# sisl/NeRFSafetyValidation

Measured on AMD Instinct MI355X. Metric: rendered_samples_per_sec, higher is better.
Workload: dtype f16; 1 GPU; Stonehenge 800x800 synthetic, hashgrid L=16 F=2 T=2^19 + ffmlp(64,2)/(64,3), fp16, occupancy-grid ray marching (run_cuda eval path, BASELINE configs[1]); rays_per_frame=640000, bound=2, cascade=2, frames_in_flight=3, fused_reference_rounding=True, parallelism=single GPU, rccl_ranks=1

## Files before the change

include/ngp_hip.h:

```cpp
#ifndef NGP_HIP_H
#define NGP_HIP_H

#include <stddef.h>
#include <stdint.h>

#ifdef __cplusplus
extern "C" {
#endif

#define NGP_OK 0
#define NGP_EINVAL (-1)
#define NGP_ELAUNCH (-2)
#define NGP_EWORKSPACE (-3)
#define NGP_ENODEVICE (-4)

#define NGP_F32 0
#define NGP_F16 1

typedef void* ngp_stream_t;

#if defined(NGP_BUILD)
#define NGP_API __attribute__((visibility("default")))
#else
#define NGP_API
// ... 246 lines not shown

NGP_API int ngp_adam_advance_step(float* step_dev, const float* found_inf_dev, ngp_stream_t stream);
NGP_API int ngp_adam_step_dev(float* param, const float* grad, float* exp_avg, float* exp_avg_sq, uint64_t n, float lr, float beta1,
                      float beta2, float eps, const float* step_dev, const float* grad_scale_dev, const float* found_inf_dev,
                      ngp_stream_t stream);

NGP_API size_t ngp_sift_workspace(uint32_t H, uint32_t W);
NGP_API size_t ngp_sift_layer_offset(uint32_t H, uint32_t W, int octave, int index);
NGP_API int ngp_sift_octaves(uint32_t H, uint32_t W);
NGP_API int ngp_sift_interest_mask(const uint8_t* rgb, uint32_t H, uint32_t W, uint32_t kernel_size, uint32_t dil_iter, uint8_t* points,
                                   uint8_t* mask, uint32_t* count, void* workspace, size_t workspace_bytes, ngp_stream_t stream);

NGP_API int ngp_debug_set_stamps(unsigned long long* device_buf);
NGP_API int ngp_debug_set_sample_hash(uint32_t* device_buf);
NGP_API int ngp_debug_disable_march_queue(int off);
NGP_API int ngp_debug_fused_features(const ngp_model* model, const float* xyzs, uint32_t M, int operator_rounding, uint16_t* features,
                             ngp_stream_t stream);
NGP_API int ngp_debug_set_grad_dump(float* device_buf);
NGP_API int ngp_render_ctx_set_debug(ngp_render_ctx* ctx, int enable, int flags, unsigned long long* stamps, uint32_t* sample_hash);

NGP_API int ngp_prof_enable(int on);
NGP_API int ngp_prof_reset(void);
NGP_API int ngp_prof_read(const char* name, double* total_ms, uint64_t* launches, double* units);

#ifdef __cplusplus
}
#endif
#endif
```

nerfsafetyvalidation_amd/_lib.py:

```python
import ctypes as C
import os

import torch

_HERE = os.path.dirname(os.path.abspath(__file__))
SO_PATH = os.environ.get("NGP_HIP_LIB", os.path.join(_HERE, "libngp_hip.so"))

NGP_F32, NGP_F16 = 0, 1
NGP_PREC_F16, NGP_PREC_F32, NGP_PREC_F16_REF = 0, 1, 2
NGP_EDT_INF = 0x7FFFFFFF

_vp, _u32, _f32, _int, _sz = C.c_void_p, C.c_uint32, C.c_float, C.c_int, C.c_size_t


class ModelStruct(C.Structure):
    _fields_ = [
        ("embeddings", _vp), ("offsets_host", _vp), ("L", _u32), ("S", _f32), ("H_base", _u32), ("gridtype", _u32),
        ("align_corners", _int), ("sigma_weights", _vp), ("sigma_hidden_mm", _u32), ("color_weights", _vp),
        ("color_hidden_mm", _u32), ("bound", _f32), ("density_scale", _f32), ("density_bitfield", _vp),
        ("cascade", _u32), ("grid_size", _u32), ("cell_tables", _vp), ("cell_levels", _u32), ("packed_weights", _vp),
        ("precision", _u32),
    ]


# ... 85 lines not shown
    "ngp_transmittance_weights": [_vp, _vp, _vp, _u32, _u32, _f32, _vp, _vp],
    "ngp_transmittance_weights_backward": [_vp, _vp, _vp, _vp, _u32, _u32, _f32, _vp, _vp],
    "ngp_sample_pdf": [_vp, _vp, _u32, _u32, _vp, _int, _u32, _vp, _vp],
    "ngp_merge_sorted": [_vp, _vp, _u32, _u32, _u32, _vp, _vp, _vp],
    "ngp_mark_untrained_grid": [_vp, _u32, _f32, _f32, _f32, _f32, _f32, _u32, _u32, _vp, _vp, _sz, _vp],
    "ngp_density_grid_points": [_vp, _u32, _u32, _f32, _vp, _vp, _vp, _vp],
    "ngp_density_grid_workspace": [_u32, _u32],
    "ngp_density_grid_update": [_vp, _u32, _u32, _u32, _vp, _vp, _u32, _f32, _f32, _vp, _sz, _vp],
    "ngp_density_grid_finish": [_vp, _u32, _u32, _f32, _vp, _vp, _vp, _sz, _vp],
    "ngp_render_uniform": [C.POINTER(ModelStruct), _vp, _vp, _vp, _vp, _u32, _u32, _vp, _vp, _vp, _vp, _vp, _u32, _vp, _vp, _u32, _vp],
    "ngp_render_upsample": [C.POINTER(ModelStruct), _vp, _vp, _vp, _vp, _u32, _u32, _u32, _vp, _vp, _vp, _vp, _vp, _vp, _u32, _vp, _vp, _u32, _vp, _sz, _vp],
    "ngp_render_upsample_workspace": [_u32, _u32, _u32],
    "ngp_debug_set_stamps": [_vp],
    "ngp_debug_set_sample_hash": [_vp],
    "ngp_debug_disable_march_queue": [_int],
    "ngp_render_ctx_set_debug": [_vp, _int, _int, _vp, _vp],
    "ngp_debug_set_grad_dump": [_vp],
    "ngp_debug_fused_features": [C.POINTER(ModelStruct), _vp, _u32, _int, _vp, _vp],
    "ngp_prof_enable": [_int],
    "ngp_prof_reset": [],
    "ngp_prof_read": [C.c_char_p, C.POINTER(C.c_double), C.POINTER(C.c_uint64), C.POINTER(C.c_double)],
}
_RESTYPES = {"ngp_render_uniform_backward_lds": _sz, "ngp_cell_tables_bytes": _sz, "ngp_packed_weights_bytes": _sz, "ngp_packed_weights_bwd_bytes": _sz, "ngp_grid_encode_backward_workspace": _sz,
             "ngp_ffmlp_backward_workspace": _sz, "ngp_ffmlp_backward_buffer_bytes": _sz, "ngp_render_upsample_workspace": _sz, "ngp_density_grid_workspace": _sz, "ngp_last_error": C.c_char_p, "ngp_march_rays_train_workspace": _sz, "ngp_uq_stats_workspace": _sz, "ngp_occupancy_lin_bytes": _sz, "ngp_edt_sq_workspace": _sz, "ngp_sift_workspace": _sz, "ngp_sift_layer_offset": _sz}

_lib = None


def lib():
    global _lib
# ... 59 lines not shown
```

nerfsafetyvalidation_amd/csrc/fused_net.hpp:

```cpp
#pragma once
#include <hip/hip_fp16.h>
#include <math.h>

#include "ngp_common.hpp"

namespace ngp {

typedef _Float16 half8 __attribute__((ext_vector_type(8)));
typedef _Float16 half2v __attribute__((ext_vector_type(2)));
typedef _Float16 half4 __attribute__((ext_vector_type(4)));
typedef float f32x4 __attribute__((ext_vector_type(4)));

struct LevelTab {
    float scale[16];
    uint32_t offset[16], size[16];
    uint32_t a1[16], a2[16];
    uint32_t mask[16];
    uint32_t flags[16];
    uint32_t cell_off[16], cell_res[16];
};

struct NetArgs {
    const uint32_t* table;
    const _Float16* packed;
// ... 859 lines not shown
struct DebugState {
    int flags = 0;
    unsigned long long* stamps = nullptr;
    uint32_t* sample_hash = nullptr;
    bool coarse_off() const { return (flags & 2) != 0; }
    bool sort_off() const { return (flags & 4) != 0; }
    bool lin_off() const { return (flags & 8) != 0; }
    bool jump_off() const { return (flags & 1) != 0; }
    bool spec_off() const { return (flags & 256) != 0; }
    bool tile_off() const { return (flags & 8192) != 0; }
    bool pre_verdict_off() const { return (flags & 16384) != 0; }
    bool narrow_items_off() const { return (flags & 32768) != 0; }
    bool prefix_replay_off() const { return (flags & 65536) != 0; }
    bool wave_march_off() const { return (flags & 131072) != 0; }
    bool cell_runs_off() const { return (flags & 262144) != 0; }
    uint32_t spec_safety_x2() const { return ((uint32_t)flags >> 9) & 15u; }
    uint32_t shrink() const { return ((uint32_t)flags >> 4) & 15u; }
};
DebugState debug_snapshot();
float* grad_dump();
bool needs_generic(const GridLevels& lv);
int fill_net(const ngp_model* m, const DebugState& dbg, const _Float16* packed, NetArgs& na, GridLevels& lv);
size_t weights_bytes(const NetArgs& na);
uint32_t resident_blocks(size_t lds);
int net_variant(const NetArgs& na, const GridLevels& lv);
bool bwd_shape_ok(const NetArgs& na);
#define NGP_WITH_NET(variant, ...)                                           \
    switch (variant) {                                                       \
        case 0: { using NET = NetF16<0>; __VA_ARGS__; } break;               \
        case 1: { using NET = NetF16<1>; __VA_ARGS__; } break;               \
// ... 10 lines not shown
```

nerfsafetyvalidation_amd/csrc/ngp_common.hpp:

```cpp
#pragma once
#include <hip/hip_runtime.h>
#include <stdint.h>
#include <stdio.h>
#include <string>

#include "../../include/ngp_hip.h"

namespace ngp {

void set_error(const char* fmt, ...);
int check_launch(const char* what);

#define NGP_REQUIRE(cond, ...)                 \
    do {                                       \
        if (!(cond)) {                         \
            ngp::set_error(__VA_ARGS__);       \
            return NGP_EINVAL;                 \
        }                                      \
    } while (0)

struct ProfScope {
    ProfScope(const char* name, hipStream_t s, double units);
    ~ProfScope();
    int slot;
// ... 8 lines not shown

constexpr int kMaxLevels = 32;
struct GridLevels {
    float scale[kMaxLevels];
    uint32_t resolution[kMaxLevels];
    uint32_t offset[kMaxLevels + 1];
    uint32_t mul1[kMaxLevels], mul2[kMaxLevels];
    uint8_t hashed[kMaxLevels], mode[kMaxLevels];
};
void fill_levels(GridLevels& lv, const int32_t* offsets_host, uint32_t L, float S, uint32_t H, uint32_t D, uint32_t gridtype,
                 bool align_corners);

__global__ void k_build_linear(const uint8_t* __restrict__ bitfield, uint32_t cascade, uint32_t logH, uint32_t* __restrict__ lin);
__global__ void k_build_coarse_linear(const unsigned long long* __restrict__ bitfield64, uint32_t cascade, uint32_t logH,
                                      unsigned long long* __restrict__ coarse);
constexpr size_t kTrainLinBytes = 1u << 20;
constexpr size_t kTrainCoarseBytes = 8192;

__device__ __forceinline__ _Float16 mul_round_f16(float w, _Float16 g) {
    float p = w * (float)g;
    asm volatile("" : "+v"(p));
    return (_Float16)p;
}
__device__ __forceinline__ float clampf(float x, float lo, float hi) { return fminf(hi, fmaxf(lo, x)); }
__device__ __forceinline__ float signf(float x) { return copysignf(1.0f, x); }

__device__ __forceinline__ uint32_t expand_bits(uint32_t v) {
    v = (v * 0x00010001u) & 0xFF0000FFu;
    v = (v * 0x00000101u) & 0x0F00F00Fu;
    v = (v * 0x00000011u) & 0xC30C30C3u;
    v = (v * 0x00000005u) & 0x49249249u;
    return v;
}
__device__ __forceinline__ uint32_t morton3D(uint32_t x, uint32_t y, uint32_t z) {
    return expand_bits(x) | (expand_bits(y) << 1) | (expand_bits(z) << 2);
}
__device__ __forceinline__ uint32_t expand_bits10(uint32_t v) {
    v = (v | (v << 16)) & 0xFF0000FFu;
    v = (v | (v << 8)) & 0x0F00F00Fu;
    v = (v | (v << 4)) & 0xC30C30C3u;
    v = (v | (v << 2)) & 0x49249249u;
    return v;
}
__device__ __forceinline__ uint32_t morton3D_cell(uint32_t x, uint32_t y, uint32_t z) {
    return expand_bits10(x) | (expand_bits10(y) << 1) | (expand_bits10(z) << 2);
}
__device__ __forceinline__ uint32_t morton3D_invert(uint32_t x) {
    x = x & 0x49249249u;
    x = (x | (x >> 2)) & 0xc30c30c3u;
    x = (x | (x >> 4)) & 0x0f00f00fu;
    x = (x | (x >> 8)) & 0xff0000ffu;
    x = (x | (x >> 16)) & 0x0000ffffu;
    return x;
}

struct Pcg32 {
    uint64_t state, inc;
    __host__ __device__ uint32_t next_uint() {
        const uint64_t old = state;
// ... 28 lines not shown
};

struct Dda {
    float ox, oy, oz, dx, dy, dz, rdx, rdy, rdz;
    float bound, rbound, dt_gamma, dt_min, dt_max, dt_c, rH, H3f, Cf, Hf, Hm1, halfH;
    double Hd;
    bool h_pow2, const_dt;
    int level_dt0;
    float t_fast_min;
    const uint32_t* grid_lin;
    uint32_t logH;
    int sx, sy, sz;
    float two_rH;
    float jump_guard;
    bool block_jump;
    const uint8_t* grid;

    __device__ __forceinline__ void init(const float* o, const float* d, const uint8_t* g, float bound_, float dt_gamma_,
                                         uint32_t max_steps, uint32_t C, uint32_t H) {
        ox = o[0]; oy = o[1]; oz = o[2];
        dx = d[0]; dy = d[1]; dz = d[2];
        rdx = 1 / dx; rdy = 1 / dy; rdz = 1 / dz;
        rH = 1 / (float)H;
        H3f = (float)(H * H * H);
        bound = bound_; rbound = 1 / bound_; dt_gamma = dt_gamma_;
        const float SQRT3 = 1.7320508075688772f;
        dt_min = 2 * SQRT3 / (float)max_steps;
        dt_max = 2 * SQRT3 * (float)(1 << (C - 1)) / (float)H;
        Cf = (float)C; Hf = (float)H; Hm1 = (float)(H - 1); Hd = (double)H;
        h_pow2 = (H & (H - 1)) == 0;
        halfH = 0.5f * Hf;
        grid = g;
        const_dt = dt_gamma_ == 0.0f;
        dt_c = fminf(dt_max, fmaxf(0.0f, dt_min));
        level_dt0 = mip_from_dt(dt_c);
        const uint32_t b = __float_as_uint(dt_c);
        const uint32_t m = (b & 0x7FFFFFu) | 0x800000u;
        t_fast_min = __uint_as_float(((b >> 23) + (uint32_t)__ffs((int)m) + 1u) << 23);
    }

    __device__ __forceinline__ void init_lin(const uint32_t* lin, uint32_t logH_, bool block_jump_) {
        grid_lin = lin;
        block_jump = block_jump_;
        logH = logH_;
        sx = (int)((__float_as_uint(dx) >> 31) ^ 1u);
        sy = (int)((__float_as_uint(dy) >> 31) ^ 1u);
        sz = (int)((__float_as_uint(dz) >> 31) ^ 1u);
        two_rH = 2.0f * rH;
        jump_guard = bound * 9.5367431640625e-7f;
    }

    __device__ __forceinline__ void skip_const_dt(float& t, float tt) const {
        const float t1 = t + dt_c;
        if (!(t1 < tt)) { t = t1; return; }
        const float d = t1 - t;
        const float r = tt - t1;
        float t2 = fmaf(ceilf(r * __builtin_amdgcn_rcpf(d)), d, t1);
        if (t2 < tt) t2 += d;
// ... 52 lines not shown
        mip_bound = use_pw ? pw : bound;
        const float mip_rbound = use_pw ? __uint_as_float((uint32_t)(127 - level) << 23) : rbound;
        nx = cell_pow2(x, mip_rbound); ny = cell_pow2(y, mip_rbound); nz = cell_pow2(z, mip_rbound);
    }
    __device__ __forceinline__ uint32_t coarse_index_lin(int level, int nx, int ny, int nz) const {
        const uint32_t lb = logH - 2;
        return ((uint32_t)level << (3 * lb)) + ((((uint32_t)nz >> 2) << (2 * lb)) | (((uint32_t)ny >> 2) << lb) | ((uint32_t)nx >> 2));
    }
    __device__ __forceinline__ bool coarse_empty_at_lin(float t, const uint32_t* coarse) const {
        float x, y, z, dt, mip_bound;
        int level, nx, ny, nz;
        locate_lin(t, x, y, z, dt, level, mip_bound, nx, ny, nz);
        const uint32_t ci = coarse_index_lin(level, nx, ny, nz);
        return ((coarse[ci >> 5] >> (ci & 31u)) & 1u) == 0;
    }
    __device__ __forceinline__ bool jump_block(float& t, float x, float y, float z, int level, float mip_bound, int nx, int ny, int nz) const {
        const float bx = fmaf((float)((nx & ~3) + 4 * sx), two_rH, -1.0f), by = fmaf((float)((ny & ~3) + 4 * sy), two_rH, -1.0f),
                    bz = fmaf((float)((nz & ~3) + 4 * sz), two_rH, -1.0f);
        if (level > level_dt0) {
            if (mip_bound != (float)(1 << level)) return false;
            const float cell4 = 4.0f * two_rH;
            const float ox_ = sx ? bx - cell4 : bx, oy_ = sy ? by - cell4 : by, oz_ = sz ? bz - cell4 : bz;
            const float mx = (ox_ <= 0.0f && ox_ + cell4 >= 0.0f) ? 0.0f : fminf(fabsf(ox_), fabsf(ox_ + cell4));
            const float my = (oy_ <= 0.0f && oy_ + cell4 >= 0.0f) ? 0.0f : fminf(fabsf(oy_), fabsf(oy_ + cell4));
            const float mz = (oz_ <= 0.0f && oz_ + cell4 >= 0.0f) ? 0.0f : fminf(fabsf(oz_), fabsf(oz_ + cell4));
            if (fmaxf(mx, fmaxf(my, mz)) < 0.5f) return false;
        }
        const float tx = fmaf(bx, mip_bound, -x) * rdx, ty = fmaf(by, mip_bound, -y) * rdy, tz = fmaf(bz, mip_bound, -z) * rdz;
        const float tmin = fminf(tx, fminf(ty, tz));
        const float tt = t + fmaxf(0.0f, tmin);
        const float t1 = t + dt_c;
        if (!(t1 < tt)) return false;
        const float d = t1 - t;
        float t2 = fmaf(ceilf((tt - t1) * __builtin_amdgcn_rcpf(d)), d, t1);
        if (t2 < tt) t2 += d;
        else if (t2 - d >= tt) t2 -= d;
        const float ex = fabsf(rdx) * jump_guard, ey = fabsf(rdy) * jump_guard, ez = fabsf(rdz) * jump_guard;
        const float em = tmin == tx ? ex : (tmin == ty ? ey : ez);
        const float lim = tmin + em;
        float ga = em;
        if (tx - ex <= lim) ga = fmaxf(ga, ex);
        if (ty - ey <= lim) ga = fmaxf(ga, ey);
        if (tz - ez <= lim) ga = fmaxf(ga, ez);
        const float guard = fmaf(t2, 9.5367431640625e-7f, ga);
        const bool clear = (t2 - tt) > guard && (tt - (t2 - d)) > guard;
        const bool same_binade = ((__float_as_uint(t2) ^ __float_as_uint(t)) >> 23) == 0;
        if (!(clear && same_binade && t >= t_fast_min)) return false;
        t = t2;
        return true;
    }

    __device__ __forceinline__ bool probe_lin(float& t, float& x, float& y, float& z, float& dt, const uint32_t* coarse,
                                              float* occupied_until = nullptr) const {
        float mip_bound;
        int level, nx, ny, nz;
        locate_lin(t, x, y, z, dt, level, mip_bound, nx, ny, nz);
        const uint32_t ci = coarse_index_lin(level, nx, ny, nz);
        bool occ = false;
        if ((coarse[ci >> 5] >> (ci & 31u)) & 1u) {
            const uint32_t fi = ((uint32_t)level << (3 * logH)) + (((uint32_t)nz << (2 * logH)) | ((uint32_t)ny << logH) | (uint32_t)nx);
            occ = ((grid_lin[fi >> 5] >> (fi & 31u)) & 1u) != 0;
            if (occ && occupied_until) {
                const float tx = fmaf(fmaf((float)(nx + sx), two_rH, -1.0f), mip_bound, -x) * rdx;
                const float ty = fmaf(fmaf((float)(ny + sy), two_rH, -1.0f), mip_bound, -y) * rdy;
                const float tz = fmaf(fmaf((float)(nz + sz), two_rH, -1.0f), mip_bound, -z) * rdz;
                const float tt = t + fminf(tx, fminf(ty, tz));
                const float g = fmaf(tt, 9.5367431640625e-7f, (fabsf(rdx) + fabsf(rdy) + fabsf(rdz)) * jump_guard);
                const float until = tt - g;
                *occupied_until = until > t ? until : t;
            }
        } else if (const_dt && block_jump && jump_block(t, x, y, z, level, mip_bound, nx, ny, nz)) {
            return false;
        }
        if (!occ) {
            const float tx = fmaf(fmaf((float)(nx + sx), two_rH, -1.0f), mip_bound, -x) * rdx;
            const float ty = fmaf(fmaf((float)(ny + sy), two_rH, -1.0f), mip_bound, -y) * rdy;
            const float tz = fmaf(fmaf((float)(nz + sz), two_rH, -1.0f), mip_bound, -z) * rdz;
            const float tt = t + fmaxf(0.0f, fminf(tx, fminf(ty, tz)));
            if (const_dt) {
                skip_const_dt(t, tt);
            } else {
                do { t += clampf(t * dt_gamma, dt_min, dt_max); } while (t < tt);
            }
        }
        return occ;
    }

// ... 33 lines not shown
```

nerfsafetyvalidation_amd/csrc/render_fused.hip:

```cpp
#include <hip/hip_fp16.h>
#include <math.h>
#include <string.h>

#include <atomic>

#include "fused_net.hpp"

namespace ngp {

constexpr int kWaves = 8;
constexpr int kThreads = kWaves * 64;
constexpr int kWavesPerSimd = 4;
constexpr int kCh = 2;
constexpr int kSlots = 64 * kCh;
constexpr size_t kLinMaxBytes = 4u << 20;
constexpr size_t kCoarseMaxBytes = 8192;
constexpr int kLookahead = 4;
constexpr int kRing = 8;

struct Ctl {
    uint32_t n_alive, n_step, step, done;
    uint32_t iters, last_n_alive, last_n_step, pad;
    unsigned long long samples_marched, samples_slots;
    uint32_t spec, rollbacks, backoff, rsv;
// ... 37 lines not shown
    lin[w] = out;
}

__global__ void __launch_bounds__(256) k_build_coarse_linear(const unsigned long long* __restrict__ bitfield64, uint32_t cascade, uint32_t logH,
                                                             unsigned long long* __restrict__ coarse) {
    const uint32_t i = blockIdx.x * 256 + threadIdx.x;
    const uint32_t lb = logH - 2, per_level = 1u << (3 * lb), B1 = (1u << lb) - 1;
    bool any = false;
    if (i < cascade * per_level) {
        const uint32_t level = i / per_level, r = i % per_level;
        const uint32_t bx = r & B1, by = (r >> lb) & B1, bz = r >> (2 * lb);
        any = bitfield64[(size_t)level * per_level + morton3D_cell(bx, by, bz)] != 0ull;
    }
    const unsigned long long m = __ballot(any);
    if ((threadIdx.x & 63) == 0 && i < cascade * per_level) coarse[i >> 6] = m;
}

struct RenderArgs {
    const float *rays_o, *rays_d, *fars;
    float* rays_t;
    float *weights_sum, *depth, *image;
    float *last_sigmas, *last_rgbs;
    float pad_sigma, pad_r, pad_g, pad_b;
    float4* dump_rec;
    uint32_t* dump_iter;
    const int32_t* alive_in;
    int32_t* staging;
    uint32_t* chunk_count;
    uint32_t sort_slow;
    Ctl* ctl;
    QueueHeads* heads;
    unsigned long long* stat_shards;
    uint32_t* death_shards;
    float4* backup;
    const uint8_t* bitfield;
    uint32_t cascade, grid_size, max_steps, perturb;
    float dt_gamma;
    Pcg32 rng;
    const uint32_t* coarse;
    uint32_t coarse_words;
    const uint32_t* bitfield_lin;
    uint32_t log_grid;
    uint32_t block_jump;
    uint32_t* sample_hash;
    unsigned long long* stamps;
    float2* march_samples;
    uint8_t* march_counts;
    uint32_t wave_slots;
    uint32_t n_rays;
    uint32_t pre_verdict;
    uint32_t wave_march_max;
    uint32_t cell_runs;
};

__host__ __device__ __forceinline__ uint32_t item_width(uint32_t n_alive, uint32_t wave_slots) {
    return n_alive >= 64u * wave_slots ? 64u : (n_alive >= 32u * wave_slots ? 32u : 16u);
}
__device__ __forceinline__ void truncate_launch(Ctl& c, const uint32_t* exhausted, uint32_t N) {
// ... 32 lines not shown
    } else {
        const size_t row = (size_t)entry * n_step + k;
        ra.last_sigmas[row] = sg;
        ra.last_rgbs[row * 3] = r; ra.last_rgbs[row * 3 + 1] = g; ra.last_rgbs[row * 3 + 2] = b;
    }
}

__device__ __forceinline__ void march_ahead_wave(const RenderArgs& ra, float bound, const Ctl& ctl, const uint32_t* coarse) {
    const uint32_t lane = threadIdx.x & 63u;
    const uint32_t entry = blockIdx.x * 4u + (threadIdx.x >> 6);
    if (entry >= ctl.n_alive) return;
    const uint32_t n_step = ctl.n_step, spec = ctl.spec;
    const int32_t ray = ra.alive_in[entry];
    Dda dda;
    dda.init(ra.rays_o + (size_t)ray * 3, ra.rays_d + (size_t)ray * 3, ra.bitfield, bound, 0.0f, ra.max_steps, ra.cascade, ra.grid_size);
    dda.init_lin(ra.bitfield_lin, ra.log_grid, ra.block_jump != 0);
    const float t_c = ra.rays_t[ray], far = ra.fars[ray];
    float t_march = t_c;
    if (ra.perturb) {
        Pcg32 rng = ra.rng;
        rng.advance((int64_t)entry);
        t_march += dda.dt_min * rng.next_float();
    }
    float last_m = t_march, geo_tc = t_c;
    uint32_t emitted = 0, rounds = 0;
    float2* out = ra.march_samples + ((size_t)(entry >> 6) * n_step) * 64 + (entry & 63u);
    while (t_march < far && emitted < n_step) {
        rounds++;
        const float t1 = t_march + dda.dt_c, d = t1 - t_march;
        const float p = lane == 0 ? t_march : fmaf((float)lane, d, t_march);
        const bool exact = t_march >= dda.t_fast_min && ((__float_as_uint(p) ^ __float_as_uint(t_march)) >> 23) == 0;
// ... 57 lines not shown
    const bool by_wave = LIN && n_alive <= ra.wave_march_max;
    if (blockIdx.x * (by_wave ? 4u : 256u) >= n_alive) return;
    __shared__ uint32_t coarse_lds[kCoarseMaxBytes / 4];
    for (uint32_t i = threadIdx.x; i < ra.coarse_words; i += blockDim.x) coarse_lds[i] = ra.coarse[i];
    __syncthreads();
    const uint32_t* coarse = ra.coarse_words ? coarse_lds : nullptr;
    if (LIN && by_wave) {
        march_ahead_wave(ra, bound, ctl, coarse);
        return;
    }
    const uint32_t entry = blockIdx.x * blockDim.x + threadIdx.x;
    if (entry >= n_alive) return;
    const int32_t ray = ra.alive_in[entry];
    Dda dda;
    dda.init(ra.rays_o + (size_t)ray * 3, ra.rays_d + (size_t)ray * 3, ra.bitfield, bound, ra.dt_gamma, ra.max_steps, ra.cascade, ra.grid_size);
    if (LIN) dda.init_lin(ra.bitfield_lin, ra.log_grid, ra.block_jump != 0);
    const float t_c = ra.rays_t[ray], far = ra.fars[ray];
    float t_march = t_c;
    if (ra.perturb) {
        Pcg32 rng = ra.rng;
        rng.advance((int64_t)entry);
        t_march += dda.dt_min * rng.next_float();
    }
    float last_m = t_march;
    float geo_tc = t_c;
    uint32_t emitted = 0;
    float2* out = ra.march_samples + ((size_t)(entry >> 6) * n_step) * 64 + (entry & 63u);
    float x, y, z, dt;
    uint32_t probes = 0, probes_coarse_empty = 0, probes_fine_empty = 0;
    const bool run_cells = LIN && dda.const_dt && ra.cell_runs != 0;
    float occ_until = 0.0f;
    while (t_march < far && emitted < n_step) {
        probes++;
        const bool diag_ce = LIN && ra.stamps && dda.coarse_empty_at_lin(t_march, coarse);
        const uint32_t emitted_before = emitted;
        if (LIN ? dda.probe_lin(t_march, x, y, z, dt, coarse, run_cells ? &occ_until : nullptr) : dda.probe(t_march, x, y, z, dt, coarse)) {
            do {
                out[(size_t)emitted * 64] = make_float2(t_march, dt);
                t_march += dt;
                const float d1 = t_march - last_m;
                last_m = t_march;
                geo_tc += d1;
                emitted++;
                if (spec && emitted % spec == 0) {
                    t_march = geo_tc;
                    last_m = geo_tc;
                }
            } while (run_cells && t_march < occ_until && t_march < far && emitted < n_step);
        }
        if (ra.stamps && emitted == emitted_before) { if (diag_ce) probes_coarse_empty++; else probes_fine_empty++; }
    }
// ... 5 lines not shown
            mx = mx > o ? mx : o;
            sm += p2;
        }
        if ((threadIdx.x & 63u) == (uint32_t)__builtin_ctzll(__ballot(true))) {
            atomicAdd(ra.stamps + 4, (unsigned long long)mx);
            atomicAdd(ra.stamps + 5, (unsigned long long)sm);
            atomicAdd(ra.stamps + 6, 1ull);
            atomicMax(ra.stamps + 7, (unsigned long long)mx);
        }
        uint32_t ce = probes_coarse_empty, fe = probes_fine_empty;
#pragma unroll
        for (int off = 32; off > 0; off >>= 1) { ce += (uint32_t)__shfl_xor((int)ce, off, 64); fe += (uint32_t)__shfl_xor((int)fe, off, 64); }
        if ((threadIdx.x & 63u) == (uint32_t)__builtin_ctzll(__ballot(true))) {
            atomicAdd(ra.stamps + 14, (unsigned long long)ce);
            atomicAdd(ra.stamps + 15, (unsigned long long)fe);
        }
    }
    if (spec && ra.pre_verdict) {
        const uint32_t K = n_step / spec, jd = emitted < n_step ? emitted / spec : 0xFFFFFFFFu;
        const unsigned long long act = __ballot(true);
        const bool leader = (threadIdx.x & 63u) == (uint32_t)__builtin_ctzll(act);
        uint32_t* ex = ra.death_shards + (size_t)kDeathShards * kSpecK + (blockIdx.x % kDeathShards) * kSpecK;
        for (uint32_t j = 0; j < K; j++) {
            const unsigned long long b = __ballot(jd == j);
            if (leader && b) atomicAdd(&ex[j], (uint32_t)__popcll(b));
        }
    }
    bool slow = false;
    if (ra.sort_slow && emitted == n_step) slow = geo_tc < far && (LIN ? dda.coarse_empty_at_lin(geo_tc, coarse) : dda.coarse_empty_at(geo_tc, coarse));
    ra.march_counts[entry] = (uint8_t)(emitted | (slow ? 128u : 0u));
// ... 581 lines not shown
}

}

using namespace ngp;

struct ngp_render_ctx {
    uint32_t max_rays = 0;
    uint32_t frame_width = 0;
    int32_t* alive[2] = {nullptr, nullptr};
    int32_t* staging = nullptr;
    uint32_t* chunk_count = nullptr;
    float* rays_t = nullptr;
    unsigned long long* coarse = nullptr;
    uint32_t* grid_lin = nullptr;
    uint32_t* death_shards = nullptr;
    float4* backup = nullptr;
    float2* march_samples = nullptr;
    uint8_t* march_counts = nullptr;
    float4* dump_rec = nullptr;
    uint32_t* dump_iter = nullptr;
    Ctl* ctl = nullptr;
    unsigned long long* stat_shards = nullptr;
    QueueHeads* heads = nullptr;
    _Float16* packed = nullptr;
    unsigned long long* status = nullptr;
    unsigned long long* status_dev = nullptr;
    unsigned long long* fin = nullptr;
    unsigned long long* fin_dev = nullptr;
    uint32_t calls = 0;
// ... 25 lines not shown
    const size_t chunks = div_up(max_rays, 64);
    bool ok = true;
    int cus = 256;
    {
        int dev = 0;
        hipDeviceProp_t prop;
        if (hipGetDevice(&dev) == hipSuccess && hipGetDeviceProperties(&prop, dev) == hipSuccess) cus = prop.multiProcessorCount;
    }
    const size_t max_items = items_bound(max_rays, (uint32_t)cus * 16u) + 8;
    ok &= hipMalloc(&c->alive[0], (size_t)max_rays * 4) == hipSuccess;
    ok &= hipMalloc(&c->alive[1], (size_t)max_rays * 4) == hipSuccess;
    ok &= hipMalloc(&c->staging, chunks * 64 * 4) == hipSuccess;
    ok &= hipMalloc(&c->chunk_count, (max_items > (size_t)div_up(max_rays, 256) ? max_items : (size_t)div_up(max_rays, 256)) * 4) == hipSuccess;
    ok &= hipMalloc(&c->rays_t, (size_t)max_rays * 4) == hipSuccess;
    ok &= hipMalloc(&c->coarse, kCoarseMaxBytes) == hipSuccess;
    ok &= hipMalloc(&c->ctl, 2 * sizeof(Ctl)) == hipSuccess;
    ok &= hipMalloc(&c->stat_shards, kStatShards * sizeof(unsigned long long)) == hipSuccess;
    ok &= hipMalloc(&c->death_shards, 2 * (size_t)kDeathWords * sizeof(uint32_t)) == hipSuccess;
    ok &= hipMalloc(&c->backup, (size_t)max_rays * 2 * sizeof(float4)) == hipSuccess;
    ok &= hipMalloc(&c->march_samples, ((size_t)max_rays + 512) * 8 * sizeof(float2)) == hipSuccess;
    ok &= hipMalloc(&c->march_counts, (size_t)max_rays) == hipSuccess;
    ok &= hipMalloc(&c->heads, 2 * sizeof(QueueHeads)) == hipSuccess;
    ok &= hipMalloc(&c->packed, (size_t)(sig_halfs(2) + sig_halfs(3)) * 2) == hipSuccess;
    ok &= hipHostMalloc(&c->status, kRing * sizeof(unsigned long long), hipHostMallocMapped | hipHostMallocCoherent) == hipSuccess;
    if (ok) {
        memset(c->status, 0, kRing * sizeof(unsigned long long));
        ok &= hipHostGetDevicePointer((void**)&c->status_dev, c->status, 0) == hipSuccess;
    }
    ok &= hipHostMalloc(&c->fin, 4 * sizeof(unsigned long long), hipHostMallocMapped | hipHostMallocCoherent) == hipSuccess;
    if (ok) {
// ... 11 lines not shown
    }
    *out = c;
    return NGP_OK;
}

int ngp_render_ctx_set_frame_width(ngp_render_ctx* ctx, uint32_t width) {
    NGP_REQUIRE(ctx, "render_ctx_set_frame_width: null context");
    ctx->frame_width = width;
    return NGP_OK;
}

int ngp_render_ctx_destroy(ngp_render_ctx* c) {
    if (!c) return NGP_OK;
    (void)hipDeviceSynchronize();
    (void)hipFree(c->alive[0]); (void)hipFree(c->alive[1]); (void)hipFree(c->staging); (void)hipFree(c->chunk_count);
    (void)hipFree(c->rays_t); (void)hipFree(c->coarse); (void)hipFree(c->grid_lin); (void)hipFree(c->death_shards); (void)hipFree(c->backup); (void)hipFree(c->march_samples); (void)hipFree(c->march_counts); (void)hipFree(c->dump_rec); (void)hipFree(c->dump_iter); (void)hipFree(c->ctl); (void)hipFree(c->stat_shards); (void)hipFree(c->heads); (void)hipFree(c->packed);
    if (c->status) (void)hipHostFree(c->status);
    if (c->fin) (void)hipHostFree(c->fin);
    for (int i = 0; i < kRing; i++) (void)hipEventDestroy(c->ev[i]);
    delete c;
    return NGP_OK;
}

static std::atomic<int> g_active_renders{0};
struct ActiveRender {
    ActiveRender() { g_active_renders.fetch_add(1, std::memory_order_relaxed); }
    ~ActiveRender() { g_active_renders.fetch_sub(1, std::memory_order_relaxed); }
};

int ngp_render_rays(ngp_render_ctx* ctx, const ngp_model* model, const float* rays_o, const float* rays_d, const float* nears,
                    const float* fars, uint32_t N, float dt_gamma, uint32_t max_steps, uint32_t perturb, float* weights_sum, float* depth,
// ... 62 lines not shown
    const uint32_t Hg = model->grid_size;
    uint32_t logH = 0;
    while ((1u << logH) < Hg) logH++;
    bool lin = use_coarse && !dbg.lin_off() && (1u << logH) == Hg && Hg >= 8 && cells / 8 <= kLinMaxBytes;
    if (lin && !ctx->grid_lin && hipMalloc(&ctx->grid_lin, kLinMaxBytes) != hipSuccess) lin = false;
    if (lin) {
        const uint32_t n_words = (uint32_t)(cells / 32), n_coarse = (uint32_t)(cells / 64);
        k_build_linear<<<div_up(n_words, 256), 256, 0, s>>>(model->density_bitfield, model->cascade, logH, ctx->grid_lin);
        k_build_coarse_linear<<<div_up(n_coarse, 256), 256, 0, s>>>((const unsigned long long*)model->density_bitfield, model->cascade, logH,
                                                                     ctx->coarse);
        ra.coarse = (const uint32_t*)ctx->coarse;
        ra.coarse_words = (uint32_t)(coarse_bytes / 4);
        ra.bitfield_lin = ctx->grid_lin;
        ra.log_grid = logH;
        ra.block_jump = dbg.jump_off() ? 0u : 1u;
    } else if (use_coarse) {
        const uint32_t n_words = (uint32_t)(cells / 64);
        k_build_coarse<<<div_up(n_words, 256), 256, 0, s>>>((const unsigned long long*)model->density_bitfield, n_words, ctx->coarse);
        ra.coarse = (const uint32_t*)ctx->coarse;
        ra.coarse_words = (uint32_t)(coarse_bytes / 4);
    } else {
        ra.sort_slow = 0;
    }
    if ((ra.sort_slow || tile_w) && last_sigmas) {
        if (!ctx->dump_rec) {
            if (hipMalloc(&ctx->dump_rec, (size_t)ctx->max_rays * 8 * sizeof(float4)) != hipSuccess ||
                hipMalloc(&ctx->dump_iter, (size_t)ctx->max_rays * 4) != hipSuccess) {
                set_error("render_rays: cannot allocate the per-ray record buffer");
                return NGP_ENODEVICE;
            }
// ... 139 lines not shown
        if (stats_host) {
            stats_host->samples_marched = fin.samples_marched;
            stats_host->samples_slots = fin.samples_slots;
            stats_host->iterations = fin.iters;
            stats_host->rays = N;
            stats_host->last_n_alive = fin.last_n_alive;
            stats_host->last_n_step = fin.last_n_step;
            stats_host->launches = launches;
            stats_host->replayed = fin.rollbacks;
            prof_add_units("k_render_iter", (double)fin.samples_marched);
        }
    }
    return NGP_OK;
}

int ngp_render_ctx_set_debug(ngp_render_ctx* ctx, int enable, int flags, unsigned long long* stamps, uint32_t* sample_hash) {
    NGP_REQUIRE(ctx, "render_ctx_set_debug: null context");
    ctx->has_debug = enable != 0;
    ctx->debug_flags = flags;
    ctx->debug_stamps = stamps;
    ctx->debug_sample_hash = sample_hash;
    return NGP_OK;
}

}
```

Measured before the change: 7.621 billion samples/s.

## Add empty-space radius map for wide block jumps in constant-dt ray marching

After: 7.581 billion samples/s. Within noise of the previous version (-0.5%).

```diff
diff --git a/include/ngp_hip.h b/include/ngp_hip.h
--- a/include/ngp_hip.h
+++ b/include/ngp_hip.h
@@ -284,6 +284,8 @@
 NGP_API int ngp_debug_set_stamps(unsigned long long* device_buf);
 NGP_API int ngp_debug_set_sample_hash(uint32_t* device_buf);
 NGP_API int ngp_debug_disable_march_queue(int off);
+NGP_API int ngp_debug_empty_radius(const uint8_t* bitfield, uint32_t cascade, uint32_t grid_size, uint8_t* radius, int on_host,
+                                   ngp_stream_t stream);
 NGP_API int ngp_debug_fused_features(const ngp_model* model, const float* xyzs, uint32_t M, int operator_rounding, uint16_t* features,
                              ngp_stream_t stream);
 NGP_API int ngp_debug_set_grad_dump(float* device_buf);
diff --git a/nerfsafetyvalidation_amd/_lib.py b/nerfsafetyvalidation_amd/_lib.py
--- a/nerfsafetyvalidation_amd/_lib.py
+++ b/nerfsafetyvalidation_amd/_lib.py
@@ -123,6 +123,7 @@
     "ngp_debug_set_stamps": [_vp],
     "ngp_debug_set_sample_hash": [_vp],
     "ngp_debug_disable_march_queue": [_int],
+    "ngp_debug_empty_radius": [_vp, _u32, _u32, _vp, _int, _vp],
     "ngp_render_ctx_set_debug": [_vp, _int, _int, _vp, _vp],
     "ngp_debug_set_grad_dump": [_vp],
     "ngp_debug_fused_features": [C.POINTER(ModelStruct), _vp, _u32, _int, _vp, _vp],
diff --git a/nerfsafetyvalidation_amd/csrc/fused_net.hpp b/nerfsafetyvalidation_amd/csrc/fused_net.hpp
--- a/nerfsafetyvalidation_amd/csrc/fused_net.hpp
+++ b/nerfsafetyvalidation_amd/csrc/fused_net.hpp
@@ -897,6 +897,7 @@
     bool prefix_replay_off() const { return (flags & 65536) != 0; }
     bool wave_march_off() const { return (flags & 131072) != 0; }
     bool cell_runs_off() const { return (flags & 262144) != 0; }
+    bool wide_jump_off() const { return (flags & 524288) != 0; }
     uint32_t spec_safety_x2() const { return ((uint32_t)flags >> 9) & 15u; }
     uint32_t shrink() const { return ((uint32_t)flags >> 4) & 15u; }
 };
diff --git a/nerfsafetyvalidation_amd/csrc/ngp_common.hpp b/nerfsafetyvalidation_amd/csrc/ngp_common.hpp
--- a/nerfsafetyvalidation_amd/csrc/ngp_common.hpp
+++ b/nerfsafetyvalidation_amd/csrc/ngp_common.hpp
@@ -46,6 +46,60 @@
 __global__ void k_build_linear(const uint8_t* __restrict__ bitfield, uint32_t cascade, uint32_t logH, uint32_t* __restrict__ lin);
 __global__ void k_build_coarse_linear(const unsigned long long* __restrict__ bitfield64, uint32_t cascade, uint32_t logH,
                                       unsigned long long* __restrict__ coarse);
+constexpr int kEmptyRadiusMax = 7;
+__host__ __device__ __forceinline__ uint32_t radius_row_bits(const uint32_t* coarse, uint32_t level, uint32_t lb, uint32_t by, uint32_t bz) {
+    const uint32_t B = 1u << lb;
+    const uint32_t base = (level << (3 * lb)) + (((bz << lb) | by) << lb);
+    uint32_t row = (coarse[base >> 5] >> (base & 31u)) & (uint32_t)((1ull << B) - 1ull);
+    if (level > 0 && 4u * (by + 1u) > B && 4u * by < 3u * B && 4u * (bz + 1u) > B && 4u * bz < 3u * B) {
+        const uint32_t lo = B / 4u, hi = (3u * B + 3u) / 4u;
+        row |= (uint32_t)(((1ull << hi) - 1ull) & ~((1ull << lo) - 1ull));
+    }
+    return row;
+}
+__host__ __device__ __forceinline__ uint32_t radius_row_dist(uint32_t row, uint32_t lb, uint32_t bx) {
+    const uint32_t B = 1u << lb, cap = (uint32_t)kEmptyRadiusMax + 1u;
+    if ((row >> bx) & 1u) return 0u;
+    const uint32_t below = row & ((1u << bx) - 1u), above = (row >> bx) >> 1;
+    const uint32_t dl = below ? bx - (31u - (uint32_t)__builtin_clz(below)) : bx + 1u;
+    const uint32_t dr = above ? (uint32_t)__builtin_ctz(above) + 1u : B - bx;
+    const uint32_t d = dl < dr ? dl : dr;
+    return d < cap ? d : cap;
+}
+__host__ __device__ __forceinline__ uint32_t radius_pass_xy(const uint32_t* coarse, uint32_t lb, uint32_t i) {
+    const uint32_t B1 = (1u << lb) - 1u, cap = (uint32_t)kEmptyRadiusMax + 1u;
+    const uint32_t level = i >> (3 * lb), bx = i & B1, by = (i >> lb) & B1, bz = (i >> (2 * lb)) & B1;
+    uint32_t best = cap;
+    for (int k = -kEmptyRadiusMax; k <= kEmptyRadiusMax; k++) {
+        const uint32_t ak = (uint32_t)(k < 0 ? -k : k);
+        const int y = (int)by + k;
+        uint32_t c = ak;
+        if (y >= 0 && y <= (int)B1) {
+            const uint32_t dx = radius_row_dist(radius_row_bits(coarse, level, lb, (uint32_t)y, bz), lb, bx);
+            c = dx > ak ? dx : ak;
+        }
+        best = c < best ? c : best;
+    }
+    return best;
+}
+__host__ __device__ __forceinline__ uint32_t radius_pass_z(const uint8_t* xy, uint32_t lb, uint32_t i) {
+    const uint32_t B1 = (1u << lb) - 1u, cap = (uint32_t)kEmptyRadiusMax + 1u;
+    const uint32_t bz = (i >> (2 * lb)) & B1;
+    uint32_t best = cap;
+    for (int k = -kEmptyRadiusMax; k <= kEmptyRadiusMax; k++) {
+        const uint32_t ak = (uint32_t)(k < 0 ? -k : k);
+        const int z = (int)bz + k;
+        uint32_t c = ak;
+        if (z >= 0 && z <= (int)B1) {
+            const uint32_t d = xy[(size_t)((int)i + k * (int)(1u << (2 * lb)))];
+            c = d > ak ? d : ak;
+        }
+        best = c < best ? c : best;
+    }
+    return best ? best - 1u : 0u;
+}
+__global__ void k_build_radius_xy(const uint32_t* __restrict__ coarse, uint32_t cascade, uint32_t logH, uint8_t* __restrict__ xy);
+__global__ void k_build_radius_z(const uint8_t* __restrict__ xy, uint32_t cascade, uint32_t logH, uint32_t* __restrict__ radius);
 constexpr size_t kTrainLinBytes = 1u << 20;
 constexpr size_t kTrainCoarseBytes = 8192;
 
@@ -67,14 +121,14 @@
 __device__ __forceinline__ uint32_t morton3D(uint32_t x, uint32_t y, uint32_t z) {
     return expand_bits(x) | (expand_bits(y) << 1) | (expand_bits(z) << 2);
 }
-__device__ __forceinline__ uint32_t expand_bits10(uint32_t v) {
+__host__ __device__ __forceinline__ uint32_t expand_bits10(uint32_t v) {
     v = (v | (v << 16)) & 0xFF0000FFu;
     v = (v | (v << 8)) & 0x0F00F00Fu;
     v = (v | (v << 4)) & 0xC30C30C3u;
     v = (v | (v << 2)) & 0x49249249u;
     return v;
 }
-__device__ __forceinline__ uint32_t morton3D_cell(uint32_t x, uint32_t y, uint32_t z) {
+__host__ __device__ __forceinline__ uint32_t morton3D_cell(uint32_t x, uint32_t y, uint32_t z) {
     return expand_bits10(x) | (expand_bits10(y) << 1) | (expand_bits10(z) << 2);
 }
 __device__ __forceinline__ uint32_t morton3D_invert(uint32_t x) {
@@ -133,6 +187,7 @@
     float two_rH;
     float jump_guard;
     bool block_jump;
+    const uint32_t* radius;
     const uint8_t* grid;
 
     __device__ __forceinline__ void init(const float* o, const float* d, const uint8_t* g, float bound_, float dt_gamma_,
@@ -158,9 +213,10 @@
         t_fast_min = __uint_as_float(((b >> 23) + (uint32_t)__ffs((int)m) + 1u) << 23);
     }
 
-    __device__ __forceinline__ void init_lin(const uint32_t* lin, uint32_t logH_, bool block_jump_) {
+    __device__ __forceinline__ void init_lin(const uint32_t* lin, uint32_t logH_, bool block_jump_, const uint32_t* radius_ = nullptr) {
         grid_lin = lin;
         block_jump = block_jump_;
+        radius = radius_;
         logH = logH_;
         sx = (int)((__float_as_uint(dx) >> 31) ^ 1u);
         sy = (int)((__float_as_uint(dy) >> 31) ^ 1u);
@@ -243,12 +299,14 @@
         const uint32_t ci = coarse_index_lin(level, nx, ny, nz);
         return ((coarse[ci >> 5] >> (ci & 31u)) & 1u) == 0;
     }
-    __device__ __forceinline__ bool jump_block(float& t, float x, float y, float z, int level, float mip_bound, int nx, int ny, int nz) const {
-        const float bx = fmaf((float)((nx & ~3) + 4 * sx), two_rH, -1.0f), by = fmaf((float)((ny & ~3) + 4 * sy), two_rH, -1.0f),
-                    bz = fmaf((float)((nz & ~3) + 4 * sz), two_rH, -1.0f);
+    __device__ __forceinline__ bool jump_block(float& t, float x, float y, float z, int level, float mip_bound, int nx, int ny, int nz,
+                                               int R = 0) const {
+        const int lo = 4 * R, span = 4 + 8 * R;
+        const float bx = fmaf((float)((nx & ~3) - lo + span * sx), two_rH, -1.0f), by = fmaf((float)((ny & ~3) - lo + span * sy), two_rH, -1.0f),
+                    bz = fmaf((float)((nz & ~3) - lo + span * sz), two_rH, -1.0f);
         if (level > level_dt0) {
             if (mip_bound != (float)(1 << level)) return false;
-            const float cell4 = 4.0f * two_rH;
+            const float cell4 = (float)span * two_rH;
             const float ox_ = sx ? bx - cell4 : bx, oy_ = sy ? by - cell4 : by, oz_ = sz ? bz - cell4 : bz;
             const float mx = (ox_ <= 0.0f && ox_ + cell4 >= 0.0f) ? 0.0f : fminf(fabsf(ox_), fabsf(ox_ + cell4));
             const float my = (oy_ <= 0.0f && oy_ + cell4 >= 0.0f) ? 0.0f : fminf(fabsf(oy_), fabsf(oy_ + cell4));
@@ -278,9 +336,20 @@
         t = t2;
         return true;
     }
+    __device__ __forceinline__ int fit_radius(int R, float t, float x, float y, float z, float mip_bound, int nx, int ny, int nz) const {
+        const float tx = fmaf(fmaf((float)((nx & ~3) + 4 * sx), two_rH, -1.0f), mip_bound, -x) * rdx;
+        const float ty = fmaf(fmaf((float)((ny & ~3) + 4 * sy), two_rH, -1.0f), mip_bound, -y) * rdy;
+        const float tz = fmaf(fmaf((float)((nz & ~3) + 4 * sz), two_rH, -1.0f), mip_bound, -z) * rdz;
+        const float tb = __uint_as_float((__float_as_uint(t) & 0x7F800000u) + 0x00800000u);
+        const float room = (tb - t) - 2.0f * dt_c;
+        const float blocks = fmaxf(fmaxf((room - tx) * fabsf(dx), (room - ty) * fabsf(dy)), (room - tz) * fabsf(dz)) *
+                             __builtin_amdgcn_rcpf(4.0f * two_rH * mip_bound);
+        const int fit = (int)fmaxf(blocks, 0.0f);
+        return fit < R ? fit : R;
+    }
 
     __device__ __forceinline__ bool probe_lin(float& t, float& x, float& y, float& z, float& dt, const uint32_t* coarse,
-                                              float* occupied_until = nullptr) const {
+                                              float* occupied_until = nullptr, uint32_t* wide_stats = nullptr) const {
         float mip_bound;
         int level, nx, ny, nz;
         locate_lin(t, x, y, z, dt, level, mip_bound, nx, ny, nz);
@@ -298,8 +367,18 @@
                 const float until = tt - g;
                 *occupied_until = until > t ? until : t;
             }
-        } else if (const_dt && block_jump && jump_block(t, x, y, z, level, mip_bound, nx, ny, nz)) {
-            return false;
+        } else if (const_dt && block_jump) {
+            int R = radius ? (int)((radius[ci >> 3] >> ((ci & 7u) * 4u)) & 15u) : 0;
+            if (R) R = fit_radius(R, t, x, y, z, mip_bound, nx, ny, nz);
+            for (;;) {
+                if (jump_block(t, x, y, z, level, mip_bound, nx, ny, nz, R)) {
+                    if (wide_stats && R) wide_stats[0]++;
+                    return false;
+                }
+                if (R == 0) break;
+                if (wide_stats) wide_stats[1]++;
+                R = 0;
+            }
         }
         if (!occ) {
             const float tx = fmaf(fmaf((float)(nx + sx), two_rH, -1.0f), mip_bound, -x) * rdx;
diff --git a/nerfsafetyvalidation_amd/csrc/render_fused.hip b/nerfsafetyvalidation_amd/csrc/render_fused.hip
--- a/nerfsafetyvalidation_amd/csrc/render_fused.hip
+++ b/nerfsafetyvalidation_amd/csrc/render_fused.hip
@@ -3,6 +3,7 @@
 #include <string.h>
 
 #include <atomic>
+#include <vector>
 
 #include "fused_net.hpp"
 
@@ -75,6 +76,20 @@
     }
     const unsigned long long m = __ballot(any);
     if ((threadIdx.x & 63) == 0 && i < cascade * per_level) coarse[i >> 6] = m;
+}
+
+__global__ void __launch_bounds__(256) k_build_radius_xy(const uint32_t* __restrict__ coarse, uint32_t cascade, uint32_t logH, uint8_t* __restrict__ xy) {
+    const uint32_t i = blockIdx.x * 256 + threadIdx.x, lb = logH - 2;
+    if (i < (cascade << (3 * lb))) xy[i] = (uint8_t)radius_pass_xy(coarse, lb, i);
+}
+__global__ void __launch_bounds__(256) k_build_radius_z(const uint8_t* __restrict__ xy, uint32_t cascade, uint32_t logH, uint32_t* __restrict__ radius) {
+    const uint32_t i = blockIdx.x * 256 + threadIdx.x, lb = logH - 2;
+    const bool in = i < (cascade << (3 * lb));
+    uint32_t v = in ? radius_pass_z(xy, lb, i) << ((i & 7u) * 4u) : 0u;
+    v |= (uint32_t)__shfl_xor((int)v, 1, 64);
+    v |= (uint32_t)__shfl_xor((int)v, 2, 64);
+    v |= (uint32_t)__shfl_xor((int)v, 4, 64);
+    if (in && (i & 7u) == 0) radius[i >> 3] = v;
 }
 
 struct RenderArgs {
@@ -103,6 +118,7 @@
     const uint32_t* bitfield_lin;
     uint32_t log_grid;
     uint32_t block_jump;
+    const uint32_t* radius;
     uint32_t* sample_hash;
     unsigned long long* stamps;
     float2* march_samples;
@@ -165,7 +181,7 @@
     const int32_t ray = ra.alive_in[entry];
     Dda dda;
     dda.init(ra.rays_o + (size_t)ray * 3, ra.rays_d + (size_t)ray * 3, ra.bitfield, bound, 0.0f, ra.max_steps, ra.cascade, ra.grid_size);
-    dda.init_lin(ra.bitfield_lin, ra.log_grid, ra.block_jump != 0);
+    dda.init_lin(ra.bitfield_lin, ra.log_grid, ra.block_jump != 0, ra.radius);
     const float t_c = ra.rays_t[ray], far = ra.fars[ray];
     float t_march = t_c;
     if (ra.perturb) {
@@ -253,7 +269,7 @@
     const int32_t ray = ra.alive_in[entry];
     Dda dda;
     dda.init(ra.rays_o + (size_t)ray * 3, ra.rays_d + (size_t)ray * 3, ra.bitfield, bound, ra.dt_gamma, ra.max_steps, ra.cascade, ra.grid_size);
-    if (LIN) dda.init_lin(ra.bitfield_lin, ra.log_grid, ra.block_jump != 0);
+    if (LIN) dda.init_lin(ra.bitfield_lin, ra.log_grid, ra.block_jump != 0, ra.radius);
     const float t_c = ra.rays_t[ray], far = ra.fars[ray];
     float t_march = t_c;
     if (ra.perturb) {
@@ -267,13 +283,14 @@
     float2* out = ra.march_samples + ((size_t)(entry >> 6) * n_step) * 64 + (entry & 63u);
     float x, y, z, dt;
     uint32_t probes = 0, probes_coarse_empty = 0, probes_fine_empty = 0;
+    uint32_t wide[2] = {0, 0};
     const bool run_cells = LIN && dda.const_dt && ra.cell_runs != 0;
     float occ_until = 0.0f;
     while (t_march < far && emitted < n_step) {
         probes++;
         const bool diag_ce = LIN && ra.stamps && dda.coarse_empty_at_lin(t_march, coarse);
         const uint32_t emitted_before = emitted;
-        if (LIN ? dda.probe_lin(t_march, x, y, z, dt, coarse, run_cells ? &occ_until : nullptr) : dda.probe(t_march, x, y, z, dt, coarse)) {
+        if (LIN ? dda.probe_lin(t_march, x, y, z, dt, coarse, run_cells ? &occ_until : nullptr, ra.stamps ? wide : nullptr) : dda.probe(t_march, x, y, z, dt, coarse)) {
             do {
                 out[(size_t)emitted * 64] = make_float2(t_march, dt);
                 t_march += dt;
@@ -309,6 +326,13 @@
         if ((threadIdx.x & 63u) == (uint32_t)__builtin_ctzll(__ballot(true))) {
             atomicAdd(ra.stamps + 14, (unsigned long long)ce);
             atomicAdd(ra.stamps + 15, (unsigned long long)fe);
+        }
+        uint32_t wt = wide[0], wr = wide[1];
+#pragma unroll
+        for (int off = 32; off > 0; off >>= 1) { wt += (uint32_t)__shfl_xor((int)wt, off, 64); wr += (uint32_t)__shfl_xor((int)wr, off, 64); }
+        if ((wt | wr) && (threadIdx.x & 63u) == (uint32_t)__builtin_ctzll(__ballot(true))) {
+            atomicAdd(ra.stamps + 12, (unsigned long long)wt);
+            atomicAdd(ra.stamps + 13, (unsigned long long)wr);
         }
     }
     if (spec && ra.pre_verdict) {
@@ -920,6 +944,8 @@
     float* rays_t = nullptr;
     unsigned long long* coarse = nullptr;
     uint32_t* grid_lin = nullptr;
+    uint32_t* radius = nullptr;
+    uint8_t* radius_xy = nullptr;
     uint32_t* death_shards = nullptr;
     float4* backup = nullptr;
     float2* march_samples = nullptr;
@@ -975,6 +1001,8 @@
     ok &= hipMalloc(&c->chunk_count, (max_items > (size_t)div_up(max_rays, 256) ? max_items : (size_t)div_up(max_rays, 256)) * 4) == hipSuccess;
     ok &= hipMalloc(&c->rays_t, (size_t)max_rays * 4) == hipSuccess;
     ok &= hipMalloc(&c->coarse, kCoarseMaxBytes) == hipSuccess;
+    ok &= hipMalloc(&c->radius, kCoarseMaxBytes * 4) == hipSuccess;
+    ok &= hipMalloc(&c->radius_xy, kCoarseMaxBytes * 8) == hipSuccess;
     ok &= hipMalloc(&c->ctl, 2 * sizeof(Ctl)) == hipSuccess;
     ok &= hipMalloc(&c->stat_shards, kStatShards * sizeof(unsigned long long)) == hipSuccess;
     ok &= hipMalloc(&c->death_shards, 2 * (size_t)kDeathWords * sizeof(uint32_t)) == hipSuccess;
@@ -1016,7 +1044,7 @@
     if (!c) return NGP_OK;
     (void)hipDeviceSynchronize();
     (void)hipFree(c->alive[0]); (void)hipFree(c->alive[1]); (void)hipFree(c->staging); (void)hipFree(c->chunk_count);
-    (void)hipFree(c->rays_t); (void)hipFree(c->coarse); (void)hipFree(c->grid_lin); (void)hipFree(c->death_shards); (void)hipFree(c->backup); (void)hipFree(c->march_samples); (void)hipFree(c->march_counts); (void)hipFree(c->dump_rec); (void)hipFree(c->dump_iter); (void)hipFree(c->ctl); (void)hipFree(c->stat_shards); (void)hipFree(c->heads); (void)hipFree(c->packed);
+    (void)hipFree(c->rays_t); (void)hipFree(c->coarse); (void)hipFree(c->radius); (void)hipFree(c->radius_xy); (void)hipFree(c->grid_lin); (void)hipFree(c->death_shards); (void)hipFree(c->backup); (void)hipFree(c->march_samples); (void)hipFree(c->march_counts); (void)hipFree(c->dump_rec); (void)hipFree(c->dump_iter); (void)hipFree(c->ctl); (void)hipFree(c->stat_shards); (void)hipFree(c->heads); (void)hipFree(c->packed);
     if (c->status) (void)hipHostFree(c->status);
     if (c->fin) (void)hipHostFree(c->fin);
     for (int i = 0; i < kRing; i++) (void)hipEventDestroy(c->ev[i]);
@@ -1109,6 +1137,12 @@
         ra.bitfield_lin = ctx->grid_lin;
         ra.log_grid = logH;
         ra.block_jump = dbg.jump_off() ? 0u : 1u;
+        static const bool no_wide = getenv("NGP_NO_WIDE_JUMP") != nullptr;
+        if (ra.block_jump && dt_gamma == 0.0f && !no_wide && !dbg.wide_jump_off()) {
+            k_build_radius_xy<<<div_up(n_coarse, 256), 256, 0, s>>>((const uint32_t*)ctx->coarse, model->cascade, logH, ctx->radius_xy);
+            k_build_radius_z<<<div_up(n_coarse, 256), 256, 0, s>>>(ctx->radius_xy, model->cascade, logH, ctx->radius);
+            ra.radius = ctx->radius;
+        }
     } else if (use_coarse) {
         const uint32_t n_words = (uint32_t)(cells / 64);
         k_build_coarse<<<div_up(n_words, 256), 256, 0, s>>>((const unsigned long long*)model->density_bitfield, n_words, ctx->coarse);
@@ -1278,6 +1312,44 @@
     return NGP_OK;
 }
 
+int ngp_debug_empty_radius(const uint8_t* bitfield, uint32_t cascade, uint32_t grid_size, uint8_t* radius, int on_host, ngp_stream_t stream) {
+    NGP_REQUIRE(bitfield && radius, "debug_empty_radius: null pointer");
+    uint32_t logH = 0;
+    while ((1u << logH) < grid_size) logH++;
+    const size_t cells = (size_t)cascade * grid_size * grid_size * grid_size;
+    NGP_REQUIRE(cascade >= 1 && grid_size >= 8 && (1u << logH) == grid_size && cells / 64 / 8 <= kCoarseMaxBytes && ((uintptr_t)bitfield & 7) == 0,
+                "debug_empty_radius: needs a power-of-two grid of 8^3 to %zu cells in all and an 8-byte aligned bitfield", kCoarseMaxBytes * 512);
+    const uint32_t n = (uint32_t)(cells / 64), lb = logH - 2, B1 = (1u << lb) - 1;
+    if (on_host) {
+        std::vector<uint32_t> coarse((n + 31) / 32, 0u);
+        std::vector<uint8_t> xy(n);
+        const unsigned long long* w = (const unsigned long long*)bitfield;
+        for (uint32_t i = 0; i < n; i++) {
+            const uint32_t level = i >> (3 * lb), r = i & ((1u << (3 * lb)) - 1);
+            if (w[((size_t)level << (3 * lb)) + morton3D_cell(r & B1, (r >> lb) & B1, r >> (2 * lb))] != 0ull) coarse[i >> 5] |= 1u << (i & 31u);
+        }
+        for (uint32_t i = 0; i < n; i++) xy[i] = (uint8_t)radius_pass_xy(coarse.data(), lb, i);
+        memset(radius, 0, n / 2);
+        for (uint32_t i = 0; i < n; i++) radius[i >> 1] |= (uint8_t)(radius_pass_z(xy.data(), lb, i) << ((i & 1u) * 4u));
+        return NGP_OK;
+    }
+    hipStream_t s = (hipStream_t)stream;
+    unsigned long long* coarse = nullptr;
+    uint8_t* xy = nullptr;
+    if (hipMalloc(&coarse, kCoarseMaxBytes) != hipSuccess || hipMalloc(&xy, n) != hipSuccess) {
+        (void)hipFree(coarse);
+        set_error("debug_empty_radius: allocation failed");
+        return NGP_ENODEVICE;
+    }
+    k_build_coarse_linear<<<div_up(n, 256), 256, 0, s>>>((const unsigned long long*)bitfield, cascade, logH, coarse);
+    k_build_radius_xy<<<div_up(n, 256), 256, 0, s>>>((const uint32_t*)coarse, cascade, logH, xy);
+    k_build_radius_z<<<div_up(n, 256), 256, 0, s>>>(xy, cascade, logH, (uint32_t*)radius);
+    const int rc = check_launch("debug_empty_radius");
+    (void)hipStreamSynchronize(s);
+    (void)hipFree(coarse); (void)hipFree(xy);
+    return rc;
+}
+
 int ngp_render_ctx_set_debug(ngp_render_ctx* ctx, int enable, int flags, unsigned long long* stamps, uint32_t* sample_hash) {
     NGP_REQUIRE(ctx, "render_ctx_set_debug: null context");
     ctx->has_debug = enable != 0;
```
